# antofuller/jumbo_mae_tpu

Hardware: AMD Instinct MI355X
Metric: pretrain images/sec (whole node) ViT-L/16 224 mask75% at 1/2/4/8 MI355X (higher is better)
Workload: dtype bf16; 1 GPU; model=vit_large_patch16 jumbo-MAE (3 CLS, shared jumbo MLP) + decoder 8x512x16h, global_batch=4096, seq_len=52, decoder_seq_len=199, parallelism=dp1, per_gpu_batch=4096, grad_accum=2, micro_batch=2048, grad_ckpt=False, hip_graph=False, optimizer=adamw(0.9,0.95) wd0.05 warmup-cosine

## Files before the change

### jumbo_mae_tpu_amd/csrc/bindings.cpp

```cpp
#include <torch/extension.h>
#include <c10/hip/HIPStream.h>
#include <hip/hip_runtime.h>

#include <climits>

#include "jm_api.h"

namespace {

hipStream_t stream() { return c10::hip::getCurrentHIPStream().stream(); }

#define CHECK_CUDA(x) TORCH_CHECK((x).is_cuda(), #x " must be a GPU tensor")
#define CHECK_CONTIG(x) TORCH_CHECK((x).is_contiguous(), #x " must be contiguous")
#define CHECK_DT(x, d) TORCH_CHECK((x).scalar_type() == (d), #x " has wrong dtype")

const uint16_t* bf(const torch::Tensor& t) { return reinterpret_cast<const uint16_t*>(t.data_ptr()); }
uint16_t* bfm(torch::Tensor& t) { return reinterpret_cast<uint16_t*>(t.data_ptr()); }
uint16_t* bfp(const torch::Tensor& t) { return reinterpret_cast<uint16_t*>(t.data_ptr()); }
const float* fopt(const c10::optional<torch::Tensor>& t) {
  return t.has_value() && t->defined() ? t->data_ptr<float>() : nullptr;
}
float* fopt_m(c10::optional<torch::Tensor>& t) { return t.has_value() && t->defined() ? t->data_ptr<float>() : nullptr; }

void check_rc(int rc, const char* what) { TORCH_CHECK(rc == 0, what, ": unsupported shape (rc=", rc, ")"); }
// ... 767 lines not shown
}

std::vector<torch::Tensor> gelu_drop(torch::Tensor a, c10::optional<torch::Tensor> b, torch::Tensor seed, double rate) {
  CHECK_CONTIG(a);
  CHECK_DT(a, torch::kBFloat16);
  check_seed(seed, a);
  TORCH_CHECK(a.numel() % 8 == 0, "gelu_drop: numel % 8");
  const auto kp = keep_params(rate);
  if (b.has_value() && b->defined()) {
    CHECK_CONTIG((*b));
    TORCH_CHECK(b->sizes() == a.sizes() && b->scalar_type() == torch::kBFloat16, "gelu_drop: (g, gp) pair");
    check_rc(jm_gelu_drop(nullptr, bfm(a), bfm(*b), a.numel(), seed.data_ptr<int64_t>(), kp.first, kp.second,
                          stream()),
             "gelu_drop");
    return {a, *b};
  }
  auto g = torch::empty_like(a), gp = torch::empty_like(a);
  check_rc(jm_gelu_drop(bf(a), bfm(g), bfm(gp), a.numel(), seed.data_ptr<int64_t>(), kp.first, kp.second, stream()),
           "gelu_drop");
  return {g, gp};
}

std::vector<torch::Tensor> softmax_dropout_fwd(torch::Tensor z, torch::Tensor seed, double rate) {
  CHECK_CONTIG(z);
  CHECK_DT(z, torch::kFloat32);
  check_seed(seed, z);
  auto [thr, scale] = keep_params(rate);
  const int S = z.size(-1);
  auto p = torch::empty_like(z);
  auto pd = torch::empty_like(z);
  check_rc(jm_softmax_dropout_fwd(z.data_ptr<float>(), p.data_ptr<float>(), pd.data_ptr<float>(), z.numel() / S, S,
                                  seed.data_ptr<int64_t>(), thr, scale, stream()),
           "softmax_dropout_fwd");
  return {p, pd};
}

torch::Tensor softmax_dropout_bwd(torch::Tensor dpd, torch::Tensor p, torch::Tensor seed, double rate) {
  CHECK_CONTIG(dpd);
  CHECK_CONTIG(p);
  CHECK_DT(dpd, torch::kFloat32);
  CHECK_DT(p, torch::kFloat32);
  TORCH_CHECK(dpd.sizes() == p.sizes(), "softmax_dropout_bwd shapes");
  check_seed(seed, p);
  auto [thr, scale] = keep_params(rate);
  const int S = p.size(-1);
  auto dz = torch::empty_like(p);
  check_rc(jm_softmax_dropout_bwd(dpd.data_ptr<float>(), p.data_ptr<float>(), dz.data_ptr<float>(), p.numel() / S, S,
                                  seed.data_ptr<int64_t>(), thr, scale, stream()),
           "softmax_dropout_bwd");
  return dz;
}

void transpose_bf16(torch::Tensor src, torch::Tensor dst) {
  CHECK_CONTIG(src);
  CHECK_CONTIG(dst);
  CHECK_DT(src, torch::kBFloat16);
  CHECK_DT(dst, torch::kBFloat16);
  TORCH_CHECK(src.dim() == 2 && dst.dim() == 2 && dst.size(0) == src.size(1) && dst.size(1) == src.size(0),
              "transpose_bf16 shapes");
  check_rc(jm_transpose_bf16(bf(src), bfm(dst), src.size(0), src.size(1), stream()), "transpose_bf16");
}

void transpose_bf16_batch(torch::Tensor desc, int64_t tiles) {
  CHECK_CONTIG(desc);
  TORCH_CHECK(desc.is_cuda() && desc.scalar_type() == torch::kInt64 && desc.dim() == 2 && desc.size(1) == 6,
              "transpose_bf16_batch: desc int64 [n, 6] on the device");
  check_rc(jm_transpose_bf16_batch(reinterpret_cast<const long long*>(desc.data_ptr<int64_t>()), (int)desc.size(0),
                                   (int)tiles, stream()),
           "transpose_bf16_batch");
}

using Tensors = std::vector<torch::Tensor>;

int group_stores(const std::vector<bool>& stores, const Tensors& gs, int S, int n) {
  if (S > 1 || stores.empty()) return 0;
  int ns = 0;
  for (int p = 0; p < n; ++p) ns += p < (int)stores.size() && stores[p];
  if (ns == n) return 1;
  for (int p = 0; p < n; ++p)
    if (p < (int)stores.size() && stores[p])
      jm_zero_f32(gs[p].data_ptr<float>(), gs[p].numel(), stream());
  return 0;
}

int64_t tn_wgrad(const char* what, const std::vector<Tensors>& dys, const std::vector<Tensors>& xs, const Tensors& gs,
                 const std::vector<bool>& stores, bool segmented) {
  const int np = (int)dys.size(), max_np = segmented ? 2 : 4, max_nb = segmented ? 32 : 1;
  TORCH_CHECK(np >= 1 && np <= max_np && (int)xs.size() == np && (int)gs.size() == np, what, ": 1..", max_np,
              " problems, each with its dy, x and g");
  const int nb = (int)dys[0].size();
  TORCH_CHECK(nb >= 1 && nb <= max_nb, what, ": 1..", max_nb, " row blocks");
  const auto dev = gs[0].device();
  TORCH_CHECK(dev.is_cuda(), what, ": g must be a GPU tensor");
  TnGroup grp{};
  TnSegs segs{};
  grp.n = np;
  int64_t rows = -1, total = 0;
  for (int p = 0; p < np; ++p) {
    TORCH_CHECK((int)dys[p].size() == nb && (int)xs[p].size() == nb, what, ": block counts differ");
    const auto &d0 = dys[p][0], &x0 = xs[p][0];
    for (int i = 0; i < nb; ++i) {
      const auto &d = dys[p][i], &x = xs[p][i];
      TORCH_CHECK(d.scalar_type() == torch::kBFloat16 && x.scalar_type() == torch::kBFloat16, what,
                  ": dy and x must be bf16");
      TORCH_CHECK(d.device() == dev && x.device() == dev, what, ": dy and x must be on g's GPU");
      TORCH_CHECK(d.dim() == 2 && x.dim() == 2 && d.stride(1) == 1 && x.stride(1) == 1, what,
                  ": dy [M,N], x [M,K] with contiguous rows");
      if (rows < 0) rows = d.size(0);
      TORCH_CHECK(d.size(0) == rows && x.size(0) == rows, what, ": dy and x of every problem and block have one M");
      TORCH_CHECK(d.size(1) == d0.size(1) && x.size(1) == x0.size(1) && d.stride(0) == d0.stride(0) &&
                      x.stride(0) == x0.stride(0),
                  what, ": block shapes / strides differ");
      if (segmented) {
        segs.a[32 * p + i] = bf(d);
        segs.b[32 * p + i] = bf(x);
      }
    }
    const int64_t N = d0.size(1), K = x0.size(1);
    TORCH_CHECK(N > 0 && K > 0 && N % 256 == 0 && K % 256 == 0, what, ": N, K multiples of 256");
    const auto& g = gs[p];
    TORCH_CHECK(g.device() == dev && g.scalar_type() == torch::kFloat32 && g.is_contiguous() && g.numel() == N * K,
                what, ": g must be fp32 [N,K], contiguous, on one GPU");
    if (!segmented) {
      grp.a[p] = bf(d0);
      grp.b[p] = bf(x0);
    }
    grp.lda[p] = d0.stride(0);
    grp.ldb[p] = x0.stride(0);
    grp.N[p] = (int)N;
    grp.K[p] = (int)K;
    total += N * K;
  }
  TORCH_CHECK(rows >= 1 && rows * nb <= INT_MAX, what, ": M out of range");
  const int M = (int)(rows * nb);
  segs.rows = (int)rows;
  segs.n = nb;
  int S = 1;
  const int sps = jm_gemm_tn_plan(grp, M, &S);
  torch::Tensor part;
  if (S > 1) part = torch::empty({S * total}, gs[0].options());
  int64_t off = 0;
  for (int p = 0; p < np; ++p) {
    grp.out[p] = S > 1 ? part.data_ptr<float>() + off : gs[p].data_ptr<float>();
    off += (int64_t)S * grp.N[p] * grp.K[p];
  }
  const int all_store = group_stores(stores, gs, S, np);
  check_rc(jm_gemm_tn(grp, segmented ? &segs : nullptr, M, sps, S, stream(), all_store), what);
  if (S > 1)
    for (int p = 0; p < np; ++p)
      check_rc(jm_splitk_reduce_add(grp.out[p], gs[p].data_ptr<float>(), (long)grp.N[p] * grp.K[p], S, stream(),
                                    p < (int)stores.size() && stores[p]),
               what);
  return S;
}

int64_t gemm_tn_wgrad(torch::Tensor dy, torch::Tensor x, torch::Tensor g, bool store) {
  return tn_wgrad("gemm_tn_wgrad", {Tensors{dy}}, {Tensors{x}}, {g}, {store}, false);
}

int64_t gemm_tn_wgrad_seg(Tensors dys, Tensors xs, torch::Tensor g, bool store) {
  return tn_wgrad("gemm_tn_wgrad_seg", {dys}, {xs}, {g}, {store}, true);
}

int64_t gemm_tn_wgrad_group(Tensors dys, Tensors xs, Tensors gs, std::vector<bool> stores) {
  std::vector<Tensors> d, x;
  for (const auto& t : dys) d.push_back({t});
  for (const auto& t : xs) x.push_back({t});
  return tn_wgrad("gemm_tn_wgrad_group", d, x, gs, stores, false);
}

int64_t gemm_tn_wgrad_seg_group(std::vector<Tensors> dys, std::vector<Tensors> xs, Tensors gs,
                                std::vector<bool> stores) {
  return tn_wgrad("gemm_tn_wgrad_seg_group", dys, xs, gs, stores, true);
}

void zero_ranges(torch::Tensor base, torch::Tensor desc, int64_t blocks) {
  CHECK_CONTIG(base);
  CHECK_DT(base, torch::kFloat32);
  TORCH_CHECK(desc.is_cuda() && desc.scalar_type() == torch::kInt64 && desc.dim() == 2 && desc.size(1) == 2,
              "zero_ranges: desc int64 [n, 2] on the device");
  check_rc(jm_zero_ranges(base.data_ptr<float>(), reinterpret_cast<const long long*>(desc.data_ptr<int64_t>()),
                          (int)desc.size(0), blocks, stream()),
           "zero_ranges");
}

std::vector<torch::Tensor> residual_ln_fwd(torch::Tensor x, torch::Tensor y, c10::optional<torch::Tensor> scale,
                                           c10::optional<torch::Tensor> mask, torch::Tensor gamma,
                                           torch::Tensor beta, double eps, int64_t T0, int64_t R0,
                                           c10::optional<torch::Tensor> out, c10::optional<torch::Tensor> seed,
                                           double rate) {
  CHECK_CUDA(x);
  TORCH_CHECK(x.dim() == 3 && x.stride(2) == 1, "x must be [B,T,D] with contiguous last dim");
  CHECK_DT(x, torch::kFloat32);
  CHECK_DT(y, torch::kBFloat16);
  CHECK_CONTIG(y);
  const int B = x.size(0), T = x.size(1), D = x.size(2);
  TORCH_CHECK(R0 >= 0 && R0 < T, "residual_ln_fwd: R0");
  TORCH_CHECK(y.numel() == (long)B * (T - R0) * D, "residual_ln_fwd: y must be [B*(T-R0), D]");
  TORCH_CHECK(T0 >= 0 && T0 < T, "residual_ln_fwd: T0");
  TORCH_CHECK(R0 == 0 || out.has_value(), "residual_ln_fwd: R0 > 0 needs out (its rows t < R0 are inputs)");
  torch::Tensor x1;
  if (out) {
    CHECK_DT(*out, torch::kFloat32);
    TORCH_CHECK(out->dim() == 3 && out->size(0) == B && out->size(1) == T && out->size(2) == D && out->stride(2) == 1,
                "residual_ln_fwd: out must be [B,T,D] with contiguous last dim");
    x1 = *out;
  } else {
    x1 = torch::empty({B, T, D}, x.options());
  }
  const long R = (long)B * (T - T0);
  auto h = torch::empty({R, D}, y.options());
  auto mean = torch::empty({R}, x.options());
  auto rstd = torch::empty({R}, x.options());
  check_rc(jm_residual_ln_fwd(x.data_ptr<float>(), x.stride(0), x.stride(1), bf(y), fopt(scale), fopt(mask),
                              x1.data_ptr<float>(), x1.stride(0), x1.stride(1), bfm(h), mean.data_ptr<float>(),
                              rstd.data_ptr<float>(), B, T, T0, D, gamma.data_ptr<float>(), beta.data_ptr<float>(),
                              (float)eps, stream(), (int)R0, make_drop(seed, rate, y, 0)),
           "residual_ln_fwd");
  return {x1, h, mean, rstd};
}

py::dict debug_lines() {
  py::dict d;
  const std::pair<const char*, int (*)()> tus[] = {
      {"attention", jm_debug_line_attention}, {"dropout", jm_debug_line_dropout},
      {"augment", jm_debug_line_augment},     {"augment_chain", jm_debug_line_augment_chain},
      {"elementwise", jm_debug_line_elementwise},
      {"gemm", jm_debug_line_gemm},           {"gemm_tn", jm_debug_line_gemm_tn},
      {"layernorm", jm_debug_line_layernorm}, {"mae", jm_debug_line_mae},
      {"optim", jm_debug_line_optim}};
  for (const auto& t : tus) {
    const int line = t.second();
    if (line) d[t.first] = line;
  }
  return d;
}

void debug_selftest(int v) { jm_debug_selftest(v, stream()); }

PYBIND11_MODULE(TORCH_EXTENSION_NAME, m) {
  m.doc() = "jumbo_mae_tpu_amd CDNA4 (gfx950) HIP kernels";
  m.def("layernorm_fwd", &layernorm_fwd, py::arg("x"), py::arg("gamma"), py::arg("beta"), py::arg("eps"),
        py::arg("out_dtype"), py::arg("also_bf16") = false);
  m.def("layernorm_bwd", &layernorm_bwd, py::arg("dy"), py::arg("x"), py::arg("mean"), py::arg("rstd"),
        py::arg("gamma"), py::arg("dgamma"), py::arg("dbeta"), py::arg("accum"), py::arg("dres") = py::none(),
        py::arg("out") = py::none(), py::arg("res_y") = py::none(), py::arg("res_scale") = py::none(),
        py::arg("res_mask") = py::none(), py::arg("res_dscale") = py::none(), py::arg("res_dbias") = py::none(),
        py::arg("res_T0") = 0, py::arg("res_out") = py::none(), py::arg("res_seed") = py::none(),
        py::arg("res_rate") = 0.0, py::arg("res_ioff") = 0, py::arg("hx") = py::none(), py::arg("beta") = py::none());
  m.def("gelu_fwd", &gelu_fwd);
  m.def("dropout_apply", &dropout_apply);
  m.def("dropout_apply_", &dropout_apply_);
  m.def("rrc_resize", &rrc_resize, py::arg("src"), py::arg("tab"), py::arg("size"), py::arg("tmp_bytes"),
        py::arg("tmp_rows_max"));
  m.def("rrc_kmax", &jm_rrc_kmax);
  m.def("window_resize", &window_resize, py::arg("src"), py::arg("tab"), py::arg("size"), py::arg("tmp_bytes"),
        py::arg("tmp_rows_max"));
  m.def("window_tab", &jm_window_tab);
  m.def("aug_chain", &aug_chain, py::arg("images"), py::arg("chain"), py::arg("scratch"));
  m.def("gelu_drop", &gelu_drop, py::arg("a"), py::arg("b") = py::none(), py::arg("seed"), py::arg("rate"));
  m.def("softmax_dropout_fwd", &softmax_dropout_fwd);
  m.def("softmax_dropout_bwd", &softmax_dropout_bwd);
  m.def("gelu_bwd", &gelu_bwd, py::arg("h"), py::arg("da"), py::arg("bias_grad") = py::none(),
        py::arg("deriv") = false);
  m.def("colsum", &colsum);
  m.def("splitk_reduce_add", &splitk_reduce_add);
  m.def("residual_ln_fwd", &residual_ln_fwd, py::arg("x"), py::arg("y"), py::arg("scale"), py::arg("mask"),
        py::arg("gamma"), py::arg("beta"), py::arg("eps"), py::arg("T0"), py::arg("R0") = 0,
        py::arg("out") = py::none(), py::arg("seed") = py::none(), py::arg("rate") = 0.0);
  m.def("transpose_bf16", &transpose_bf16);
  m.def("residual_fwd", &residual_fwd, py::arg("x"), py::arg("y"), py::arg("scale"), py::arg("mask"),
        py::arg("out") = py::none(), py::arg("seed") = py::none(), py::arg("rate") = 0.0, py::arg("ioff") = 0);
  m.def("residual_bwd", &residual_bwd, py::arg("dout"), py::arg("y"), py::arg("scale"), py::arg("mask"),
        py::arg("dscale"), py::arg("ydtype"), py::arg("dbias") = py::none(), py::arg("out") = py::none(),
        py::arg("seed") = py::none(), py::arg("rate") = 0.0, py::arg("ioff") = 0);
  m.def("attn_fwd", &attn_fwd, py::arg("qkv"), py::arg("heads"), py::arg("seed") = py::none(), py::arg("rate") = 0.0);
  m.def("attn_bwd", &attn_bwd, py::arg("dO"), py::arg("qkv"), py::arg("o"), py::arg("lse"), py::arg("heads"),
        py::arg("dbias") = py::none(), py::arg("seed") = py::none(), py::arg("rate") = 0.0);
  m.def("attn_max_seq", &jm_attn_max_seq);
  m.def("attn_head_dims", &attn_head_dims);
  m.def("attn_fused_bias", &attn_fused_bias, py::arg("S"), py::arg("hd"));
  m.def("attn_dropout", &attn_dropout, py::arg("S"), py::arg("hd"));
  m.def("gemm_tn_wgrad", &gemm_tn_wgrad, py::arg("dy"), py::arg("x"), py::arg("g"), py::arg("store") = false);
  m.def("gemm_tn_wgrad_seg", &gemm_tn_wgrad_seg, py::arg("dys"), py::arg("xs"), py::arg("g"), py::arg("store") = false);
  m.def("zero_ranges", &zero_ranges, "zero float ranges of a flat buffer (one launch)");
  m.def("colsum_add_f32", &colsum_add_f32, "g += x.sum(0) for a row-strided fp32 [rows, n] view");
  m.def("gemm_tn_wgrad_seg_group", &gemm_tn_wgrad_seg_group, py::arg("dys"), py::arg("xs"), py::arg("gs"),
        py::arg("stores") = std::vector<bool>{}, "grouped segmented weight gradients (<= 2 problems)");
  m.def("gemm_tn_wgrad_group", &gemm_tn_wgrad_group, py::arg("dys"), py::arg("xs"), py::arg("gs"),
        py::arg("stores") = std::vector<bool>{}, "grouped weight gradients over one M (<= 4 problems)");
  m.def("gemm_test_force", &jm_gemm_test_force, py::arg("path"), py::arg("rows") = 0,
        "numerics tests only: NT GEMM kernel path 0 = by shape, 1 = 64-deep main loop everywhere, "
        "2 = 4-phase kernels at every M without tail split (rows = forced tile height)");
  m.def("gemm_nt_tiles", &jm_gemm_nt_tiles, py::arg("M"), py::arg("N"), py::arg("K") = 1024, py::arg("epi") = 0,
        py::arg("lda") = 0, "output tiles (workgroups before split-K) of an NT launch");
  m.def(
      "gemm_nt_tail_plan",
      [](int M, int N, int K, int epi, long lda) {
        int r = 0;
        long n = 0;
        const int S = jm_gemm_nt_tail_plan(M, N, K, epi, lda, &r, &n);
        return std::make_pair(S, r);
      },
      py::arg("M"), py::arg("N"), py::arg("K"), py::arg("epi") = 0, py::arg("lda") = 0,
      "(S, tail tiles) of the tail split of an NT launch (S = 0: none); read-only");
  m.def("transpose_bf16_batch", &transpose_bf16_batch);
  m.def("gemm_nt_splitk", &gemm_nt_splitk, py::arg("A"), py::arg("B"), py::arg("bias") = py::none(),
        py::arg("splits") = 8, py::arg("add") = py::none());
  m.def("gemm_nt_dgelu", &gemm_nt_dgelu, py::arg("A"), py::arg("B"), py::arg("pre"), py::arg("dbias") = py::none(),
        py::arg("deriv") = false, py::arg("rate") = 0.0);
  m.def("gemm_nt_f32", &gemm_nt_f32, py::arg("A"), py::arg("B"));
  m.def("gemm_nt", &gemm_nt, py::arg("A"), py::arg("B"), py::arg("bias") = py::none(), py::arg("gelu") = false,
        py::arg("gelu_only") = false, py::arg("gelu_deriv") = false, py::arg("seed") = py::none(),
        py::arg("rate") = 0.0);
  m.def("opt_sumsq", &opt_sumsq);
  m.def("opt_adamw", &opt_adamw);
  m.def("opt_lamb_phase1", &opt_lamb_phase1);
  m.def("opt_lars_norms", &opt_lars_norms);
  m.def("opt_apply_trust", &opt_apply_trust);
  m.def("opt_sgd", &opt_sgd);
  m.def("patchify_normalize", &patchify_normalize);
  m.def("gather_patches", &gather_patches);
  m.def("embed_finish", &embed_finish);
  m.def("zero_f32", &zero_f32, "fp32 zero fill kernel (the store-mode gradients' pre-reduce fill)");
  m.def("mask_ids", &mask_ids, "random-masking permutation ids + mask from noise (one workgroup per row)");
  m.def("unshuffle_fwd", &unshuffle_fwd);
  m.def("unshuffle_bwd", &unshuffle_bwd);
  m.def("patch_mse_fwd", &patch_mse_fwd);
  m.def("mix_patches", &mix_patches);
  m.def("patch_mse_bwd", &patch_mse_bwd);
  m.def("debug_lines", &debug_lines);
  m.def("debug_selftest", &debug_selftest);
#ifdef JM_DEBUG
  m.attr("debug_build") = true;
#else
  m.attr("debug_build") = false;
#endif
}
```

### jumbo_mae_tpu_amd/csrc/gemm_tn.hip

```cpp
#include <type_traits>

#include "common.h"
#include "jm_api.h"

namespace {

constexpr int TN_ = 256, TK_ = 256, BS = 32, NST = 4, NTH = 512;
constexpr int STAGE = (TN_ + TK_) * BS;

typedef __attribute__((address_space(3))) void lds_void_t;

JM_DEVICE __amdgpu_buffer_rsrc_t make_rsrc(const uint16_t* base, long bytes) {
  const int n = bytes >= 0xffffffffL ? -1 : (int)bytes;
  return __builtin_amdgcn_make_buffer_rsrc((void*)base, (short)0, n, 0x00020000);
}

JM_DEVICE void blds16(__amdgpu_buffer_rsrc_t r, uint32_t voff, uint32_t soff, uint16_t* l) {
  __builtin_amdgcn_raw_ptr_buffer_load_lds(r, (lds_void_t*)(l), 16, voff, soff, 0, 0);
}

JM_DEVICE f32x4_t mfma16(bf16x8_t a, bf16x8_t b, f32x4_t c) {
  return __builtin_amdgcn_mfma_f32_16x16x32_bf16(a, b, c, 0, 0, 0);
}

JM_DEVICE s16x4_t tr4(const uint16_t* p) {
  s16x4_t r;
  const uint32_t a = (uint32_t)(size_t)((const __attribute__((address_space(3))) uint16_t*)p);
  asm volatile("ds_read_b64_tr_b16 %0, %1" : "=v"(r) : "v"(a));
  return r;
}

template <int X, int OFF>
JM_DEVICE s16x4_t tr4x(uint32_t a) {
  s16x4_t r;
  if constexpr (X == 0) {
    asm volatile("ds_read_b64_tr_b16 %0, %1 offset:%2" : "=v"(r) : "v"(a), "i"(OFF));
  } else {
    uint32_t tmp;
    asm volatile("v_xor_b32 %1, %3, %2\n\tds_read_b64_tr_b16 %0, %1 offset:%4"
                 : "=v"(r), "=&v"(tmp) : "v"(a), "i"(X), "i"(OFF));
  }
  return r;
}

template <int N, int I = 0, typename F>
JM_DEVICE void static_for(F&& f) {
  if constexpr (I < N) {
    f(std::integral_constant<int, I>{});
    static_for<N, I + 1>(f);
  }
}

JM_DEVICE void wait_lds() {
  asm volatile("s_waitcnt lgkmcnt(0)" ::: "memory");
  __builtin_amdgcn_sched_barrier(0);
}

JM_DEVICE bf16x8_t cat44(s16x4_t lo, s16x4_t hi) {
  s16x8_t s;
  s[0] = lo[0]; s[1] = lo[1]; s[2] = lo[2]; s[3] = lo[3];
  s[4] = hi[0]; s[5] = hi[1]; s[6] = hi[2]; s[7] = hi[3];
  return __builtin_bit_cast(bf16x8_t, s);
}

template <int X, int OFF>
JM_DEVICE bf16x8_t tr8x(uint32_t a) {
  s16x4_t lo, hi;
  if constexpr (X == 0) {
    asm volatile("ds_read_b64_tr_b16 %0, %2 offset:%3\n\tds_read_b64_tr_b16 %1, %2 offset:%4"
                 : "=&v"(lo), "=v"(hi) : "v"(a), "i"(OFF), "i"(OFF + 1024));
  } else {
    uint32_t tmp;
    asm volatile("v_xor_b32 %2, %4, %3\n\tds_read_b64_tr_b16 %0, %2 offset:%5\n\tds_read_b64_tr_b16 %1, %2 offset:%6"
                 : "=&v"(lo), "=&v"(hi), "=&v"(tmp) : "v"(a), "i"(X), "i"(OFF), "i"(OFF + 1024));
  }
  return cat44(lo, hi);
}

JM_DEVICE int tswz(int row) { return ((row & 3) | (((row >> 3) & 1) << 2)) << 1; }

JM_DEVICE int toff(int row, int col) { return row * 256 + ((((col >> 3) ^ tswz(row)) & 31) << 3) + (col & 7); }

struct TFrags {
  bf16x8_t b[4], a[8];
};

template <int ACC>
__global__ __launch_bounds__(NTH, 1) void gemm_tn_kernel(const uint16_t* __restrict__ A, long lda,
                                                         const uint16_t* __restrict__ B, long ldb, int M, int N,
                                                         int K, int steps_per_split, float* __restrict__ out,
                                                         long ldo, long split_stride, TnSegs segs) {
  JM_DGUARD(blockDim.x == NTH && steps_per_split >= 1 && M > 0);
  extern __shared__ __attribute__((aligned(16))) uint16_t smem[];
  const int tid = threadIdx.x;
  const int wave = __builtin_amdgcn_readfirstlane(tid >> 6), lane = tid & 63;
  const int l16 = lane & 15, g = lane >> 4;
  const int wr = wave >> 2, wc = wave & 3;

  const int nK = K / TK_;
  const int tiles = (N / TN_) * nK;
  const int nwg = gridDim.x;
  const int orig = blockIdx.x;
  const int xcd = orig & 7, q = nwg >> 3, r = nwg & 7;
  const int wg = (xcd < r ? xcd * (q + 1) : r * (q + 1) + (xcd - r) * q) + (orig >> 3);
  const int split = wg / tiles, tile = wg - split * tiles;
  const int n0 = (tile / nK) * TN_, k0 = (tile % nK) * TK_;
  const int m_begin = split * steps_per_split * BS;
  const int rows = min(M - m_begin, steps_per_split * BS);
  int nk = (rows + BS - 1) / BS;
  nk += nk & 1;
  if (nk < 2) nk = 2;

  uint32_t a_src[2], b_src[2];
#pragma unroll
  for (int rr = 0; rr < 2; ++rr) {
    const int row = rr * 16 + wave * 2 + (lane >> 5);
    const int c = (lane & 31) ^ tswz(row);
    a_src[rr] = (uint32_t)((row * lda + c * 8) * 2);
    b_src[rr] = (uint32_t)((row * ldb + c * 8) * 2);
  }
  auto issue = [&](int t) {
    uint16_t* la = smem + (t % NST) * STAGE;
    uint16_t* lb = la + BS * TN_;
    const int row = m_begin + t * BS;
    const int sg = min(row / segs.rows, segs.n - 1);
    const int loc = row - sg * segs.rows;
    const int left = row < m_begin + rows ? min(segs.rows - loc, m_begin + rows - row) : 0;
    const __amdgpu_buffer_rsrc_t sra = make_rsrc(segs.a[sg] + (long)loc * lda + n0, (long)left * lda * 2);
    const __amdgpu_buffer_rsrc_t srb = make_rsrc(segs.b[sg] + (long)loc * ldb + k0, (long)left * ldb * 2);
#pragma unroll
    for (int rr = 0; rr < 2; ++rr) {
      blds16(sra, a_src[rr], 0, la + (rr * 16 + wave * 2) * TN_);
      blds16(srb, b_src[rr], 0, lb + (rr * 16 + wave * 2) * TK_);
    }
  };
  const int r1 = 8 * g + (l16 >> 2);
  const int cl = 4 * (l16 & 3);
  auto read_one = [&](int t, TFrags& f, int i) {
    const uint16_t* la = smem + (t % NST) * STAGE;
    const uint16_t* lb = la + BS * TN_;
    if (i < 4) {
      const int col = wc * 64 + i * 16 + cl;
      f.b[i] = cat44(tr4(lb + toff(r1, col)), tr4(lb + toff(r1 + 4, col)));
    } else {
      const int col = wr * 128 + (i - 4) * 16 + cl;
      f.a[i - 4] = cat44(tr4(la + toff(r1, col)), tr4(la + toff(r1 + 4, col)));
    }
  };

  f32x4_t acc[8][4];
#pragma unroll
  for (int i = 0; i < 8; ++i)
#pragma unroll
    for (int j = 0; j < 4; ++j) acc[i][j] = f32x4_t{0.f, 0.f, 0.f, 0.f};

  auto wait_bar = [&](auto outstanding_stages) {
    constexpr int W = decltype(outstanding_stages)::value * 4;
    if constexpr (W == 8) asm volatile("s_waitcnt vmcnt(8) lgkmcnt(0)\n\ts_barrier" ::: "memory");
    if constexpr (W == 4) asm volatile("s_waitcnt vmcnt(4) lgkmcnt(0)\n\ts_barrier" ::: "memory");
    if constexpr (W == 0) asm volatile("s_waitcnt vmcnt(0) lgkmcnt(0)\n\ts_barrier" ::: "memory");
  };
  auto step = [&](auto kind, int t, TFrags& cur, TFrags& nxt) {
    constexpr int KIND = decltype(kind)::value;
    wait_lds();
    if constexpr (KIND == 3) issue(t + 3);
#pragma unroll
    for (int mt = 0; mt < 4; ++mt)
#pragma unroll
      for (int nt = 0; nt < 4; ++nt) acc[mt][nt] = mfma16(cur.b[nt], cur.a[mt], acc[mt][nt]);
    __builtin_amdgcn_sched_barrier(0);
    if constexpr (KIND > 0) wait_bar(std::integral_constant<int, KIND - 1>{});
    __builtin_amdgcn_sched_barrier(0);
#pragma unroll
    for (int i = 0; i < 16; ++i) {
      if constexpr (KIND > 0) {
        if (i < 12) read_one(t + 1, nxt, i);
      }
      const int mt = 4 + i / 4, nt = i % 4;
      acc[mt][nt] = mfma16(cur.b[nt], cur.a[mt], acc[mt][nt]);
      __builtin_amdgcn_sched_barrier(0);
    }
  };
  using K3 = std::integral_constant<int, 3>;
  using K2 = std::integral_constant<int, 2>;
  using K1 = std::integral_constant<int, 1>;
  using K0 = std::integral_constant<int, 0>;

  issue(0);
  issue(1);
  if (nk > 2) {
    issue(2);
    wait_bar(std::integral_constant<int, 2>{});
  } else {
    wait_bar(std::integral_constant<int, 1>{});
  }
  __builtin_amdgcn_sched_barrier(0);
  TFrags f0, f1;
#pragma unroll
  for (int i = 0; i < 12; ++i) read_one(0, f0, i);
  int t = 0;
  for (; t + 4 < nk; t += 2) {
    step(K3{}, t, f0, f1);
    step(K3{}, t + 1, f1, f0);
  }
  if (nk - t == 4) {
    step(K3{}, t, f0, f1);
    step(K2{}, t + 1, f1, f0);
    t += 2;
  }
  step(K1{}, t, f0, f1);
  step(K0{}, t + 1, f1, f0);

  float* dst = ACC ? out : out + (long)split * split_stride;
#pragma unroll
  for (int mt = 0; mt < 8; ++mt) {
    const int n = n0 + wr * 128 + mt * 16 + l16;
    float* row = dst + (long)n * ldo + k0 + wc * 64 + 4 * g;
#pragma unroll
    for (int nt = 0; nt < 4; ++nt) {
      float v[4] = {acc[mt][nt][0], acc[mt][nt][1], acc[mt][nt][2], acc[mt][nt][3]};
      if (ACC) {
        float o[4];
        load4(row + nt * 16, o);
#pragma unroll
        for (int i = 0; i < 4; ++i) v[i] += o[i];
      }
      store4(row + nt * 16, v);
    }
  }
}

constexpr int SLOT4 = 64 * 128;

template <int ACC, bool SEG, bool GRP = false>
__global__ __launch_bounds__(NTH, 1) void gemm_tn4_kernel(const uint16_t* __restrict__ A, long lda,
                                                          const uint16_t* __restrict__ B, long ldb, int M, int N,
                                                          int K, int steps_per_split, float* __restrict__ out,
                                                          long ldo, long split_stride, TnSegs segs = {},
                                                          TnGroup grp = {}) {
  JM_DGUARD(blockDim.x == NTH && steps_per_split >= 4 && steps_per_split % 4 == 0 && M > 0);
  extern __shared__ __attribute__((aligned(16))) uint16_t smem[];
  const int tid = threadIdx.x;
  const int wave = __builtin_amdgcn_readfirstlane(tid >> 6), lane = tid & 63;
  const int l16 = lane & 15, g = lane >> 4;
  const int wr = wave >> 2, wc = wave & 3;
  if (__builtin_amdgcn_readfirstlane(tid) >= 256) __builtin_amdgcn_s_setprio(1);

  int nK = K / TK_;
  const int tiles = GRP ? grp.tile0[grp.n] : (N / TN_) * nK;
  const int nwg = gridDim.x;
  const int orig = blockIdx.x;
  const int xcd = orig & 7, q = nwg >> 3, r = nwg & 7;
  const int wg = (xcd < r ? xcd * (q + 1) : r * (q + 1) + (xcd - r) * q) + (orig >> 3);
  const int split = wg / tiles;
  int tile = wg - split * tiles;
  int soff = 0;
  if constexpr (GRP) {
    int p = 0;
    while (p + 1 < grp.n && tile >= grp.tile0[p + 1]) ++p;
    tile -= grp.tile0[p];
    soff = 32 * p;
    A = grp.a[p];
    B = grp.b[p];
    lda = grp.lda[p];
    ldb = grp.ldb[p];
    N = grp.N[p];
    K = grp.K[p];
    out = grp.out[p];
    ldo = K;
    split_stride = (long)N * K;
    nK = K / TK_;
  }
  const int n0 = (tile / nK) * TN_, k0 = (tile % nK) * TK_;
  const int m_begin = split * steps_per_split * BS;
  const int rows = min(M - m_begin, steps_per_split * BS);
  int nk = (rows + 63) / 64;
  nk += nk & 1;

  const __amdgpu_buffer_rsrc_t ra = make_rsrc(SEG ? segs.a[soff] : A + (long)m_begin * lda + n0, SEG ? 0 : (long)rows * lda * 2);
  const __amdgpu_buffer_rsrc_t rb = make_rsrc(SEG ? segs.b[soff] : B + (long)m_begin * ldb + k0, SEG ? 0 : (long)rows * ldb * 2);
  uint32_t a_src[2][2], b_src[2][2];
#pragma unroll
  for (int rr = 0; rr < 2; ++rr) {
    const int pr = (2 * wave + rr) * 4 + (lane >> 4);
    const int c = (lane & 15) ^ tswz(pr);
#pragma unroll
    for (int h = 0; h < 2; ++h) {
      a_src[h][rr] = (uint32_t)((pr * lda + (c >> 3) * 128 + h * 64 + (c & 7) * 8) * 2);
      b_src[h][rr] = (uint32_t)((pr * ldb + (c >> 2) * 64 + h * 32 + (c & 3) * 8) * 2);
    }
  }
  auto issue = [&](int t, auto slot) {
    constexpr int S = decltype(slot)::value;
    uint16_t* l = smem + ((t & 1) * 4 + S) * SLOT4 + (2 * wave) * 4 * 128;
    if constexpr (SEG) {
      const int row = m_begin + t * 64;
      const int sg = min(row / segs.rows, segs.n - 1);
      const int loc = row - sg * segs.rows;
      const int left = row < m_begin + rows ? min(segs.rows - loc, m_begin + rows - row) : 0;
      if constexpr (S < 2) {
        const __amdgpu_buffer_rsrc_t sra = make_rsrc(segs.a[soff + sg] + (long)loc * lda + n0, (long)left * lda * 2);
#pragma unroll
        for (int rr = 0; rr < 2; ++rr) blds16(sra, a_src[S][rr], 0, l + rr * 4 * 128);
      } else {
        const __amdgpu_buffer_rsrc_t srb = make_rsrc(segs.b[soff + sg] + (long)loc * ldb + k0, (long)left * ldb * 2);
#pragma unroll
        for (int rr = 0; rr < 2; ++rr) blds16(srb, b_src[S - 2][rr], 0, l + rr * 4 * 128);
      }
    } else {
#pragma unroll
      for (int rr = 0; rr < 2; ++rr) {
        if constexpr (S < 2) blds16(ra, a_src[S][rr], (uint32_t)(t * 64 * lda * 2), l + rr * 4 * 128);
        else blds16(rb, b_src[S - 2][rr], (uint32_t)(t * 64 * ldb * 2), l + rr * 4 * 128);
      }
    }
  };
  const int qrow = 8 * g + (l16 >> 2), pp = l16 & 3;
  const int sw = tswz(qrow);
  const uint32_t lds0 = (uint32_t)(size_t)((const __attribute__((address_space(3))) uint16_t*)smem);
  const uint32_t a_lo = 2 * (qrow * 128 + (((wr * 8 + (pp >> 1)) ^ sw) << 3) + (pp & 1) * 4);
  const uint32_t b_lo = 2 * (qrow * 128 + (((wc * 4 + (pp >> 1)) ^ sw) << 3) + (pp & 1) * 4);
  constexpr bool PRE = true;
  constexpr int NA = PRE ? 4 : 1, NB = PRE ? 2 : 1;
  uint32_t a_addr[2][NA], b_addr[2][NB];
#pragma unroll
  for (int st = 0; st < 2; ++st) {
#pragma unroll
    for (int j = 0; j < NA; ++j) a_addr[st][j] = (lds0 + st * 4 * SLOT4 * 2 + a_lo) ^ (uint32_t)(j << 5);
#pragma unroll
    for (int j = 0; j < NB; ++j) b_addr[st][j] = (lds0 + st * 4 * SLOT4 * 2 + b_lo) ^ (uint32_t)(j << 5);
  }
  typedef bf16x8_t AF[4][2];
  typedef bf16x8_t BF[2][2];
  auto read_a1 = [&](int t, auto sl, AF& f, auto ic) {
    constexpr int SL = decltype(sl)::value, I = decltype(ic)::value;
    constexpr int OFF = SL * SLOT4 * 2 + (I / 4) * 32 * 256;
    if constexpr (PRE) f[I % 4][I / 4] = tr8x<0, OFF>(a_addr[t & 1][I % 4]);
    else f[I % 4][I / 4] = tr8x<(I % 4) << 5, OFF>(a_addr[t & 1][0]);
  };
  auto read_b1 = [&](int t, auto sl, BF& f, auto ic) {
    constexpr int SL = decltype(sl)::value, I = decltype(ic)::value;
    constexpr int OFF = SL * SLOT4 * 2 + (I / 2) * 32 * 256;
    if constexpr (PRE) f[I % 2][I / 2] = tr8x<0, OFF>(b_addr[t & 1][I % 2]);
    else f[I % 2][I / 2] = tr8x<(I % 2) << 5, OFF>(b_addr[t & 1][0]);
  };
  f32x4_t acc[8][4];
#pragma unroll
  for (int i = 0; i < 8; ++i)
#pragma unroll
    for (int j = 0; j < 4; ++j) acc[i][j] = f32x4_t{0.f, 0.f, 0.f, 0.f};
  auto phase = [&](auto mh, auto nh, const AF& a, const BF& b, auto nreads, auto&& rd) {
    constexpr int MH = decltype(mh)::value, NH = decltype(nh)::value, NR = decltype(nreads)::value;
    static_for<16>([&](auto ic) {
      constexpr int i = decltype(ic)::value;
      if constexpr (i < NR) rd(ic);
      constexpr int kk = i / 8, mt = (i % 8) / 2, nt = i % 2;
      acc[MH * 4 + mt][NH * 2 + nt] = mfma16(b[nt][kk], a[mt][kk], acc[MH * 4 + mt][NH * 2 + nt]);
      __builtin_amdgcn_sched_barrier(0);
    });
  };
  auto sync = [&](auto n) {
    constexpr int V = decltype(n)::value;
    if constexpr (V == 12) asm volatile("s_waitcnt vmcnt(12) lgkmcnt(0)\n\ts_barrier" ::: "memory");
    else if constexpr (V == 10) asm volatile("s_waitcnt vmcnt(10) lgkmcnt(0)\n\ts_barrier" ::: "memory");
    else if constexpr (V == 6) asm volatile("s_waitcnt vmcnt(6) lgkmcnt(0)\n\ts_barrier" ::: "memory");
    else if constexpr (V == 4) asm volatile("s_waitcnt vmcnt(4) lgkmcnt(0)\n\ts_barrier" ::: "memory");
    else if constexpr (V == 2) asm volatile("s_waitcnt vmcnt(2) lgkmcnt(0)\n\ts_barrier" ::: "memory");
    else if constexpr (V == 0) asm volatile("s_waitcnt vmcnt(0) lgkmcnt(0)\n\ts_barrier" ::: "memory");
    else asm volatile("s_waitcnt lgkmcnt(0)\n\ts_barrier" ::: "memory");
    __builtin_amdgcn_sched_barrier(0);
  };
  using I0 = std::integral_constant<int, 0>;
  using I1 = std::integral_constant<int, 1>;
  using I2 = std::integral_constant<int, 2>;
  using I3 = std::integral_constant<int, 3>;
  using I4 = std::integral_constant<int, 4>;
  using I6 = std::integral_constant<int, 6>;
  using I8 = std::integral_constant<int, 8>;
  using I10 = std::integral_constant<int, 10>;
  using I12 = std::integral_constant<int, 12>;
  using IN = std::integral_constant<int, -1>;

  AF ax, ay;
  BF bp, bq;
  auto ktile = [&](auto kind, int t, BF& b0, BF& b1) {
    constexpr int KIND = decltype(kind)::value;
    sync(std::conditional_t<KIND == 0, I4, I12>{});
    if constexpr (KIND == 2) issue(t + 2, I0{});
    phase(I0{}, I0{}, ax, b0, I4{}, [&](auto i) { read_b1(t, I3{}, b1, i); });
    sync(std::conditional_t<KIND == 0, I2, std::conditional_t<KIND == 1, I10, I12>>{});
    if constexpr (KIND == 2) issue(t + 2, I3{});
    phase(I0{}, I1{}, ax, b1, I8{}, [&](auto i) { read_a1(t, I1{}, ay, i); });
    sync(IN{});
    if constexpr (KIND == 2) issue(t + 2, I1{});
    phase(I1{}, I1{}, ay, b1, I0{}, [&](auto) {});
    if constexpr (KIND > 0) {
      sync(std::conditional_t<KIND == 1, I0, I6>{});
      if constexpr (KIND == 2) issue(t + 2, I2{});
      phase(I1{}, I0{}, ay, b0, I12{}, [&](auto i) {
        constexpr int I = decltype(i)::value;
        if constexpr (I < 8) read_a1(t + 1, I0{}, ax, i);
        else read_b1(t + 1, I2{}, b1, std::integral_constant<int, I - 8>{});
      });
    } else {
      phase(I1{}, I0{}, ay, b0, I0{}, [&](auto) {});
    }
  };
  using K2 = std::integral_constant<int, 2>;
  using K1 = std::integral_constant<int, 1>;
  using K0 = std::integral_constant<int, 0>;

  issue(0, I0{});
  issue(0, I3{});
  issue(0, I1{});
  issue(0, I2{});
  issue(1, I0{});
  issue(1, I3{});
  issue(1, I1{});
  sync(I6{});
  issue(1, I2{});
  static_for<8>([&](auto i) { read_a1(0, I0{}, ax, i); });
  static_for<4>([&](auto i) { read_b1(0, I2{}, bp, i); });
  int t = 0;
  for (; t + 4 <= nk; t += 2) {
    ktile(K2{}, t, bp, bq);
    ktile(K2{}, t + 1, bq, bp);
  }
  ktile(K1{}, t, bp, bq);
  ktile(K0{}, t + 1, bq, bp);

  float* dst = ACC ? out : out + (long)split * split_stride;
#pragma unroll
  for (int mt = 0; mt < 8; ++mt) {
    const int n = n0 + wr * 128 + mt * 16 + l16;
    float* row = dst + (long)n * ldo + k0 + wc * 64 + 4 * g;
#pragma unroll
    for (int nt = 0; nt < 4; ++nt) {
      float v[4] = {acc[mt][nt][0], acc[mt][nt][1], acc[mt][nt][2], acc[mt][nt][3]};
      if (ACC) {
        float o[4];
        load4(row + nt * 16, o);
#pragma unroll
        for (int i = 0; i < 4; ++i) v[i] += o[i];
      }
      store4(row + nt * 16, v);
    }
  }
}

}

size_t jm_gemm_tn_smem() { return (size_t)NST * STAGE * sizeof(uint16_t); }

int jm_gemm_tn_plan(const TnGroup& grp, int M, int* S_out) {
  long NK = 0;
  int tiles = 0;
  for (int p = 0; p < grp.n; ++p) {
    NK += (long)grp.N[p] * grp.K[p];
    tiles += (grp.N[p] / TN_) * (grp.K[p] / TK_);
  }
  const int steps = (M + BS - 1) / BS;
  const int unit = 4;
  double best = 1e30;
  int best_sps = (steps + unit - 1) / unit * unit, best_S = 1;
  for (int S = 1; S <= 128 && steps > 0; ++S) {
    int sps = (steps + S - 1) / S;
    sps = (sps + unit - 1) / unit * unit;
    if (sps < 4 && S > 1) break;
    const int s_eff = (steps + sps - 1) / sps;
    const long wgs = (long)tiles * s_eff;
    const long waves = (wgs + 255) / 256;
    const double t_steps = (double)waves * (sps + 12);
    const double t_red = s_eff > 1 ? (double)s_eff * NK * 8.0 / 5.0e12 * 1e6 : 0.0;
    const double est = t_steps + t_red;
    if (est < best) {
      best = est;
      best_sps = sps;
      best_S = s_eff;
    }
  }
  *S_out = best_S;
  return best_sps;
}

namespace {
template <auto KERN, typename... Args>
void tn_launch(int wgs, hipStream_t st, Args... args) {
  static const hipError_t lds = hipFuncSetAttribute((const void*)KERN, hipFuncAttributeMaxDynamicSharedMemorySize,
                                                    (int)jm_gemm_tn_smem());
  (void)lds;
  KERN<<<wgs, NTH, jm_gemm_tn_smem(), st>>>(args...);
}

template <int ACC>
void tn_dispatch(const TnGroup& grp, const TnSegs* segs, int M, int sps, int S, hipStream_t st) {
  const int wgs = grp.tile0[grp.n] * S;
  const TnSegs sg = segs ? *segs : TnSegs{};
  if (grp.n > 1) {
    if (segs)
      tn_launch<gemm_tn4_kernel<ACC, true, true>>(wgs, st, nullptr, 0, nullptr, 0, M, 0, 0, sps, nullptr, 0, 0, sg, grp);
    else
      tn_launch<gemm_tn4_kernel<ACC, false, true>>(wgs, st, nullptr, 0, nullptr, 0, M, 0, 0, sps, nullptr, 0, 0, sg, grp);
    return;
  }
  const int N = grp.N[0], K = grp.K[0];
  const long ldo = K, ss = S > 1 ? (long)N * K : 0;
  if (!segs)
    tn_launch<gemm_tn4_kernel<ACC, false, false>>(wgs, st, grp.a[0], grp.lda[0], grp.b[0], grp.ldb[0], M, N, K, sps,
                                                  grp.out[0], ldo, ss, sg, TnGroup{});
  else if (segs->rows % 64 == 0)
    tn_launch<gemm_tn4_kernel<ACC, true, false>>(wgs, st, grp.a[0], grp.lda[0], grp.b[0], grp.ldb[0], M, N, K, sps,
                                                 grp.out[0], ldo, ss, sg, TnGroup{});
// ... 28 lines not shown
```

Baseline: 6779 images/sec.

## Restructure TN weight-gradient kernel into 32-row stages with four-deep load pipeline

Rewrites the main loop of the 4-phase TN weight-gradient GEMM kernel. Each 64-row k-tile split into two half-phases becomes a sequence of 32-row stages, each doing a full 8x4 MFMA sweep. Each stage's global-to-LDS copy is issued four stages ahead, and fragment reads for the next stage are interleaved into the current stage's MFMAs at a fixed schedule. This is meant to improve overlap of loads, LDS transposed reads and MFMAs, and to cut barrier count per unit of work, at the cost of more fragment registers and a rounding of row counts to 128. It also removes the unused XOR-address variants of the transposed read helpers and adds a test-only hook to force the split size.

```diff
diff --git a/jumbo_mae_tpu_amd/csrc/bindings.cpp b/jumbo_mae_tpu_amd/csrc/bindings.cpp
--- a/jumbo_mae_tpu_amd/csrc/bindings.cpp
+++ b/jumbo_mae_tpu_amd/csrc/bindings.cpp
@@ -873,6 +873,8 @@
       jm_zero_f32(gs[p].data_ptr<float>(), gs[p].numel(), stream());
   return 0;
 }
+
+int g_tn_test_sps = 0;
 
 int64_t tn_wgrad(const char* what, const std::vector<Tensors>& dys, const std::vector<Tensors>& xs, const Tensors& gs,
                  const std::vector<bool>& stores, bool segmented) {
@@ -927,7 +929,11 @@
   segs.rows = (int)rows;
   segs.n = nb;
   int S = 1;
-  const int sps = jm_gemm_tn_plan(grp, M, &S);
+  int sps = jm_gemm_tn_plan(grp, M, &S);
+  if (g_tn_test_sps > 0) {
+    sps = g_tn_test_sps;
+    S = ((M + 31) / 32 + sps - 1) / sps;
+  }
   torch::Tensor part;
   if (S > 1) part = torch::empty({S * total}, gs[0].options());
   int64_t off = 0;
@@ -1080,6 +1086,9 @@
         py::arg("stores") = std::vector<bool>{}, "grouped segmented weight gradients (<= 2 problems)");
   m.def("gemm_tn_wgrad_group", &gemm_tn_wgrad_group, py::arg("dys"), py::arg("xs"), py::arg("gs"),
         py::arg("stores") = std::vector<bool>{}, "grouped weight gradients over one M (<= 4 problems)");
+  m.def("gemm_tn_test_force", [](int sps) { g_tn_test_sps = sps; }, py::arg("sps") = 0,
+        "numerics tests only: 32-row steps per M split of the weight-gradient launches (a multiple of 4; "
+        "0 = jm_gemm_tn_plan's choice)");
   m.def("gemm_test_force", &jm_gemm_test_force, py::arg("path"), py::arg("rows") = 0,
         "numerics tests only: NT GEMM kernel path 0 = by shape, 1 = 64-deep main loop everywhere, "
         "2 = 4-phase kernels at every M without tail split (rows = forced tile height)");
diff --git a/jumbo_mae_tpu_amd/csrc/gemm_tn.hip b/jumbo_mae_tpu_amd/csrc/gemm_tn.hip
--- a/jumbo_mae_tpu_amd/csrc/gemm_tn.hip
+++ b/jumbo_mae_tpu_amd/csrc/gemm_tn.hip
@@ -30,19 +30,6 @@
   return r;
 }
 
-template <int X, int OFF>
-JM_DEVICE s16x4_t tr4x(uint32_t a) {
-  s16x4_t r;
-  if constexpr (X == 0) {
-    asm volatile("ds_read_b64_tr_b16 %0, %1 offset:%2" : "=v"(r) : "v"(a), "i"(OFF));
-  } else {
-    uint32_t tmp;
-    asm volatile("v_xor_b32 %1, %3, %2\n\tds_read_b64_tr_b16 %0, %1 offset:%4"
-                 : "=v"(r), "=&v"(tmp) : "v"(a), "i"(X), "i"(OFF));
-  }
-  return r;
-}
-
 template <int N, int I = 0, typename F>
 JM_DEVICE void static_for(F&& f) {
   if constexpr (I < N) {
@@ -63,17 +50,11 @@
   return __builtin_bit_cast(bf16x8_t, s);
 }
 
-template <int X, int OFF>
+template <int OFF>
 JM_DEVICE bf16x8_t tr8x(uint32_t a) {
   s16x4_t lo, hi;
-  if constexpr (X == 0) {
-    asm volatile("ds_read_b64_tr_b16 %0, %2 offset:%3\n\tds_read_b64_tr_b16 %1, %2 offset:%4"
-                 : "=&v"(lo), "=v"(hi) : "v"(a), "i"(OFF), "i"(OFF + 1024));
-  } else {
-    uint32_t tmp;
-    asm volatile("v_xor_b32 %2, %4, %3\n\tds_read_b64_tr_b16 %0, %2 offset:%5\n\tds_read_b64_tr_b16 %1, %2 offset:%6"
-                 : "=&v"(lo), "=&v"(hi), "=&v"(tmp) : "v"(a), "i"(X), "i"(OFF), "i"(OFF + 1024));
-  }
+  asm volatile("ds_read_b64_tr_b16 %0, %2 offset:%3\n\tds_read_b64_tr_b16 %1, %2 offset:%4"
+               : "=&v"(lo), "=v"(hi) : "v"(a), "i"(OFF), "i"(OFF + 1024));
   return cat44(lo, hi);
 }
 
@@ -231,6 +212,11 @@
 }
 
 constexpr int SLOT4 = 64 * 128;
+
+constexpr int tn4_read_at(int i) {
+  constexpr int at[13] = {0, 1, 4, 2, 5, 3, 6, 10, 7, 11, 8, -1, 9};
+  return i % 2 == 0 && i < 26 ? at[i / 2] : -1;
+}
 
 template <int ACC, bool SEG, bool GRP = false>
 __global__ __launch_bounds__(NTH, 1) void gemm_tn4_kernel(const uint16_t* __restrict__ A, long lda,
@@ -274,45 +260,41 @@
   const int n0 = (tile / nK) * TN_, k0 = (tile % nK) * TK_;
   const int m_begin = split * steps_per_split * BS;
   const int rows = min(M - m_begin, steps_per_split * BS);
-  int nk = (rows + 63) / 64;
-  nk += nk & 1;
+  const int ns = (rows + 127) / 128 * 4;
 
   const __amdgpu_buffer_rsrc_t ra = make_rsrc(SEG ? segs.a[soff] : A + (long)m_begin * lda + n0, SEG ? 0 : (long)rows * lda * 2);
   const __amdgpu_buffer_rsrc_t rb = make_rsrc(SEG ? segs.b[soff] : B + (long)m_begin * ldb + k0, SEG ? 0 : (long)rows * ldb * 2);
-  uint32_t a_src[2][2], b_src[2][2];
-#pragma unroll
-  for (int rr = 0; rr < 2; ++rr) {
-    const int pr = (2 * wave + rr) * 4 + (lane >> 4);
+  uint32_t a_src[2], b_src[2];
+  {
+    const int pr = 4 * wave + (lane >> 4);
     const int c = (lane & 15) ^ tswz(pr);
 #pragma unroll
     for (int h = 0; h < 2; ++h) {
-      a_src[h][rr] = (uint32_t)((pr * lda + (c >> 3) * 128 + h * 64 + (c & 7) * 8) * 2);
-      b_src[h][rr] = (uint32_t)((pr * ldb + (c >> 2) * 64 + h * 32 + (c & 3) * 8) * 2);
-    }
-  }
-  auto issue = [&](int t, auto slot) {
-    constexpr int S = decltype(slot)::value;
-    uint16_t* l = smem + ((t & 1) * 4 + S) * SLOT4 + (2 * wave) * 4 * 128;
+      a_src[h] = (uint32_t)((pr * lda + (c >> 3) * 128 + h * 64 + (c & 7) * 8) * 2);
+      b_src[h] = (uint32_t)((pr * ldb + (c >> 2) * 64 + h * 32 + (c & 3) * 8) * 2);
+    }
+  }
+  auto issue = [&](int s0, auto jc) {
+    constexpr int J = decltype(jc)::value;
+    uint16_t* l = smem + (J >> 1) * 4 * SLOT4 + ((J & 1) * 32 + 4 * wave) * 128;
     if constexpr (SEG) {
-      const int row = m_begin + t * 64;
+      const int row = m_begin + (s0 + (J & 2)) * BS;
       const int sg = min(row / segs.rows, segs.n - 1);
       const int loc = row - sg * segs.rows;
       const int left = row < m_begin + rows ? min(segs.rows - loc, m_begin + rows - row) : 0;
-      if constexpr (S < 2) {
-        const __amdgpu_buffer_rsrc_t sra = make_rsrc(segs.a[soff + sg] + (long)loc * lda + n0, (long)left * lda * 2);
-#pragma unroll
-        for (int rr = 0; rr < 2; ++rr) blds16(sra, a_src[S][rr], 0, l + rr * 4 * 128);
-      } else {
-        const __amdgpu_buffer_rsrc_t srb = make_rsrc(segs.b[soff + sg] + (long)loc * ldb + k0, (long)left * ldb * 2);
-#pragma unroll
-        for (int rr = 0; rr < 2; ++rr) blds16(srb, b_src[S - 2][rr], 0, l + rr * 4 * 128);
-      }
+      const __amdgpu_buffer_rsrc_t sra = make_rsrc(segs.a[soff + sg] + (long)loc * lda + n0, (long)left * lda * 2);
+      const __amdgpu_buffer_rsrc_t srb = make_rsrc(segs.b[soff + sg] + (long)loc * ldb + k0, (long)left * ldb * 2);
+      const uint32_t oa = (uint32_t)((J & 1) * BS * lda * 2), ob = (uint32_t)((J & 1) * BS * ldb * 2);
+      blds16(sra, a_src[0], oa, l);
+      blds16(sra, a_src[1], oa, l + SLOT4);
+      blds16(srb, b_src[0], ob, l + 2 * SLOT4);
+      blds16(srb, b_src[1], ob, l + 3 * SLOT4);
     } else {
-#pragma unroll
-      for (int rr = 0; rr < 2; ++rr) {
-        if constexpr (S < 2) blds16(ra, a_src[S][rr], (uint32_t)(t * 64 * lda * 2), l + rr * 4 * 128);
-        else blds16(rb, b_src[S - 2][rr], (uint32_t)(t * 64 * ldb * 2), l + rr * 4 * 128);
-      }
+      const uint32_t oa = (uint32_t)((s0 + J) * BS * lda * 2), ob = (uint32_t)((s0 + J) * BS * ldb * 2);
+      blds16(ra, a_src[0], oa, l);
+      blds16(ra, a_src[1], oa, l + SLOT4);
+      blds16(rb, b_src[0], ob, l + 2 * SLOT4);
+      blds16(rb, b_src[1], ob, l + 3 * SLOT4);
     }
   };
   const int qrow = 8 * g + (l16 >> 2), pp = l16 & 3;
@@ -320,114 +302,85 @@
   const uint32_t lds0 = (uint32_t)(size_t)((const __attribute__((address_space(3))) uint16_t*)smem);
   const uint32_t a_lo = 2 * (qrow * 128 + (((wr * 8 + (pp >> 1)) ^ sw) << 3) + (pp & 1) * 4);
   const uint32_t b_lo = 2 * (qrow * 128 + (((wc * 4 + (pp >> 1)) ^ sw) << 3) + (pp & 1) * 4);
-  constexpr bool PRE = true;
-  constexpr int NA = PRE ? 4 : 1, NB = PRE ? 2 : 1;
-  uint32_t a_addr[2][NA], b_addr[2][NB];
+  uint32_t a_addr[2][4], b_addr[2][2];
 #pragma unroll
   for (int st = 0; st < 2; ++st) {
 #pragma unroll
-    for (int j = 0; j < NA; ++j) a_addr[st][j] = (lds0 + st * 4 * SLOT4 * 2 + a_lo) ^ (uint32_t)(j << 5);
-#pragma unroll
-    for (int j = 0; j < NB; ++j) b_addr[st][j] = (lds0 + st * 4 * SLOT4 * 2 + b_lo) ^ (uint32_t)(j << 5);
-  }
-  typedef bf16x8_t AF[4][2];
-  typedef bf16x8_t BF[2][2];
-  auto read_a1 = [&](int t, auto sl, AF& f, auto ic) {
-    constexpr int SL = decltype(sl)::value, I = decltype(ic)::value;
-    constexpr int OFF = SL * SLOT4 * 2 + (I / 4) * 32 * 256;
-    if constexpr (PRE) f[I % 4][I / 4] = tr8x<0, OFF>(a_addr[t & 1][I % 4]);
-    else f[I % 4][I / 4] = tr8x<(I % 4) << 5, OFF>(a_addr[t & 1][0]);
-  };
-  auto read_b1 = [&](int t, auto sl, BF& f, auto ic) {
-    constexpr int SL = decltype(sl)::value, I = decltype(ic)::value;
-    constexpr int OFF = SL * SLOT4 * 2 + (I / 2) * 32 * 256;
-    if constexpr (PRE) f[I % 2][I / 2] = tr8x<0, OFF>(b_addr[t & 1][I % 2]);
-    else f[I % 2][I / 2] = tr8x<(I % 2) << 5, OFF>(b_addr[t & 1][0]);
+    for (int j = 0; j < 4; ++j) a_addr[st][j] = (lds0 + st * 4 * SLOT4 * 2 + a_lo) ^ (uint32_t)(j << 5);
+#pragma unroll
+    for (int j = 0; j < 2; ++j) b_addr[st][j] = (lds0 + st * 4 * SLOT4 * 2 + b_lo) ^ (uint32_t)(j << 5);
+  }
+  bf16x8_t fa[8], fx[2], fb[2][4];
+  auto read_frag = [&](auto jc, auto ic) {
+    constexpr int J = decltype(jc)::value, I = decltype(ic)::value, MT = I - 4;
+    constexpr int ROWS = (J & 1) * 32 * 256;
+    if constexpr (I < 4) fb[J & 1][I] = tr8x<(2 + I / 2) * SLOT4 * 2 + ROWS>(b_addr[J >> 1][I % 2]);
+    else if constexpr (MT >= 6 && (J & 1)) fx[MT - 6] = tr8x<(MT / 4) * SLOT4 * 2 + ROWS>(a_addr[J >> 1][MT % 4]);
+    else fa[MT] = tr8x<(MT / 4) * SLOT4 * 2 + ROWS>(a_addr[J >> 1][MT % 4]);
   };
   f32x4_t acc[8][4];
 #pragma unroll
   for (int i = 0; i < 8; ++i)
 #pragma unroll
     for (int j = 0; j < 4; ++j) acc[i][j] = f32x4_t{0.f, 0.f, 0.f, 0.f};
-  auto phase = [&](auto mh, auto nh, const AF& a, const BF& b, auto nreads, auto&& rd) {
-    constexpr int MH = decltype(mh)::value, NH = decltype(nh)::value, NR = decltype(nreads)::value;
-    static_for<16>([&](auto ic) {
-      constexpr int i = decltype(ic)::value;
-      if constexpr (i < NR) rd(ic);
-      constexpr int kk = i / 8, mt = (i % 8) / 2, nt = i % 2;
-      acc[MH * 4 + mt][NH * 2 + nt] = mfma16(b[nt][kk], a[mt][kk], acc[MH * 4 + mt][NH * 2 + nt]);
-      __builtin_amdgcn_sched_barrier(0);
-    });
-  };
-  auto sync = [&](auto n) {
-    constexpr int V = decltype(n)::value;
-    if constexpr (V == 12) asm volatile("s_waitcnt vmcnt(12) lgkmcnt(0)\n\ts_barrier" ::: "memory");
-    else if constexpr (V == 10) asm volatile("s_waitcnt vmcnt(10) lgkmcnt(0)\n\ts_barrier" ::: "memory");
-    else if constexpr (V == 6) asm volatile("s_waitcnt vmcnt(6) lgkmcnt(0)\n\ts_barrier" ::: "memory");
-    else if constexpr (V == 4) asm volatile("s_waitcnt vmcnt(4) lgkmcnt(0)\n\ts_barrier" ::: "memory");
-    else if constexpr (V == 2) asm volatile("s_waitcnt vmcnt(2) lgkmcnt(0)\n\ts_barrier" ::: "memory");
-    else if constexpr (V == 0) asm volatile("s_waitcnt vmcnt(0) lgkmcnt(0)\n\ts_barrier" ::: "memory");
-    else asm volatile("s_waitcnt lgkmcnt(0)\n\ts_barrier" ::: "memory");
-    __builtin_amdgcn_sched_barrier(0);
-  };
   using I0 = std::integral_constant<int, 0>;
   using I1 = std::integral_constant<int, 1>;
   using I2 = std::integral_constant<int, 2>;
   using I3 = std::integral_constant<int, 3>;
-  using I4 = std::integral_constant<int, 4>;
-  using I6 = std::integral_constant<int, 6>;
-  using I8 = std::integral_constant<int, 8>;
-  using I10 = std::integral_constant<int, 10>;
-  using I12 = std::integral_constant<int, 12>;
   using IN = std::integral_constant<int, -1>;
-
-  AF ax, ay;
-  BF bp, bq;
-  auto ktile = [&](auto kind, int t, BF& b0, BF& b1) {
-    constexpr int KIND = decltype(kind)::value;
-    sync(std::conditional_t<KIND == 0, I4, I12>{});
-    if constexpr (KIND == 2) issue(t + 2, I0{});
-    phase(I0{}, I0{}, ax, b0, I4{}, [&](auto i) { read_b1(t, I3{}, b1, i); });
-    sync(std::conditional_t<KIND == 0, I2, std::conditional_t<KIND == 1, I10, I12>>{});
-    if constexpr (KIND == 2) issue(t + 2, I3{});
-    phase(I0{}, I1{}, ax, b1, I8{}, [&](auto i) { read_a1(t, I1{}, ay, i); });
-    sync(IN{});
-    if constexpr (KIND == 2) issue(t + 2, I1{});
-    phase(I1{}, I1{}, ay, b1, I0{}, [&](auto) {});
-    if constexpr (KIND > 0) {
-      sync(std::conditional_t<KIND == 1, I0, I6>{});
-      if constexpr (KIND == 2) issue(t + 2, I2{});
-      phase(I1{}, I0{}, ay, b0, I12{}, [&](auto i) {
-        constexpr int I = decltype(i)::value;
-        if constexpr (I < 8) read_a1(t + 1, I0{}, ax, i);
-        else read_b1(t + 1, I2{}, b1, std::integral_constant<int, I - 8>{});
-      });
-    } else {
-      phase(I1{}, I0{}, ay, b0, I0{}, [&](auto) {});
-    }
-  };
-  using K2 = std::integral_constant<int, 2>;
-  using K1 = std::integral_constant<int, 1>;
-  using K0 = std::integral_constant<int, 0>;
+  auto stage = [&](auto pc, auto jn) {
+    constexpr int P = decltype(pc)::value, JN = decltype(jn)::value;
+    static_for<32>([&](auto ic) {
+      constexpr int i = decltype(ic)::value;
+      if constexpr (JN >= 0 && tn4_read_at(i) >= 0) read_frag(jn, std::integral_constant<int, tn4_read_at(i)>{});
+      constexpr int mt = i / 4, nt = i % 4;
+      if constexpr (mt >= 6 && P) acc[mt][nt] = mfma16(fb[P][nt], fx[mt - 6], acc[mt][nt]);
+      else acc[mt][nt] = mfma16(fb[P][nt], fa[mt], acc[mt][nt]);
+      __builtin_amdgcn_sched_barrier(0);
+    });
+  };
+  auto sync = [&](auto n) {
+    constexpr int V = decltype(n)::value;
+    if constexpr (V == 12) asm volatile("s_waitcnt vmcnt(12) lgkmcnt(0)\n\ts_barrier" ::: "memory");
+    else if constexpr (V == 8) asm volatile("s_waitcnt vmcnt(8) lgkmcnt(0)\n\ts_barrier" ::: "memory");
+    else if constexpr (V == 4) asm volatile("s_waitcnt vmcnt(4) lgkmcnt(0)\n\ts_barrier" ::: "memory");
+    else if constexpr (V == 0) asm volatile("s_waitcnt vmcnt(0) lgkmcnt(0)\n\ts_barrier" ::: "memory");
+    else asm volatile("s_waitcnt lgkmcnt(0)" ::: "memory");
+    __builtin_amdgcn_sched_barrier(0);
+  };
+  using V12 = std::integral_constant<int, 12>;
+  using V8 = std::integral_constant<int, 8>;
+  using V4 = std::integral_constant<int, 4>;
 
   issue(0, I0{});
-  issue(0, I3{});
   issue(0, I1{});
   issue(0, I2{});
-  issue(1, I0{});
-  issue(1, I3{});
-  issue(1, I1{});
-  sync(I6{});
-  issue(1, I2{});
-  static_for<8>([&](auto i) { read_a1(0, I0{}, ax, i); });
-  static_for<4>([&](auto i) { read_b1(0, I2{}, bp, i); });
-  int t = 0;
-  for (; t + 4 <= nk; t += 2) {
-    ktile(K2{}, t, bp, bq);
-    ktile(K2{}, t + 1, bq, bp);
-  }
-  ktile(K1{}, t, bp, bq);
-  ktile(K0{}, t + 1, bq, bp);
+  issue(0, I3{});
+  sync(V12{});
+  static_for<12>([&](auto i) { read_frag(I0{}, i); });
+  int s = 0;
+  for (; s + 8 <= ns; s += 4) {
+    sync(V8{});
+    issue(s + 4, I0{});
+    stage(I0{}, I1{});
+    sync(V8{});
+    issue(s + 4, I1{});
+    stage(I1{}, I2{});
+    sync(V8{});
+    issue(s + 4, I2{});
+    stage(I0{}, I3{});
+    sync(V8{});
+    issue(s + 4, I3{});
+    stage(I1{}, I0{});
+  }
+  sync(V8{});
+  stage(I0{}, I1{});
+  sync(V4{});
+  stage(I1{}, I2{});
+  sync(I0{});
+  stage(I0{}, I3{});
+  sync(IN{});
+  stage(I1{}, IN{});
 
   float* dst = ACC ? out : out + (long)split * split_stride;
 #pragma unroll
```

Result: no change. 6829 images/sec, median of 6 (+0.7%).
